# dbry/audio-resampler

Hardware: AMD Instinct MI355X
Metric: Msamples/s (out) 44.1k->48k preset -4, 8ch float32 (higher is better)
Workload: dtype i8 x 4 digits (32-bit fixed point of the f32 samples and the fp64-blended filter rows, exact i32 accumulation, one float rounding per output)

## Files before the change

### audio_resampler_amd/csrc/fir_matrix_i8.hip

```cpp
#include "fir_matrix_stream.hip.h"
#include <atomic>
#include <cstdlib>

#if !ART_WIDE

namespace {

typedef int i32x4 __attribute__ ((ext_vector_type (4)));
typedef int i32x16 __attribute__ ((ext_vector_type (16)));

constexpr int I8_KC = 32;
constexpr int I8_PITCH = 48;
constexpr int I8_COLS = 128;
constexpr int I8_MAX_PPW = 64;
constexpr int i8_ppw (int cols, int cg) { return cols / cg > I8_MAX_PPW ? I8_MAX_PPW : cols / cg; }
constexpr float I8_SCALE = 1073741824.0f;
constexpr float I8_LIMIT = 1.98f;

struct I8Geom {
    int tr;
    int cols;
    int tiles;
    int ktot;
    int g;
    int gq4;
    int super_groups;
    int sg_per_xcd;
    unsigned char *a_planes;
    unsigned long long *a_masks;
    unsigned long long *tile_masks;
    int mask_words;
    const unsigned char *x_planes;
    unsigned int *x_planes_w;
    int eb_periods, ebs;
    int eb_blocks, eb_step;
    int b0;
    int cgrp;
    int slices;
    int slice_blocks;
    unsigned int *peaks;
    unsigned int eb_plane_bytes;
    size_t x_bytes;
    int *flag; int epoch;
    int *shifts;
    unsigned char *parts;
    int rows_cached;
    int rows_table;
    double tb_base; int tb_lin, tb_w;
    unsigned int tb_n0;
    int jr_rot;
};

__device__ __forceinline__ int shift_of_peak (unsigned int bits)
{
    const int e = max ((int)(bits >> 23), 1);
    return 157 - e - ((bits & 0x7e0000u) == 0x7e0000u ? 1 : 0);
}

constexpr int I8_STAGE_THREADS = 256;
constexpr int I8_STAGE_K = 4;

__device__ __forceinline__ unsigned int digits_of (int q) { return ((unsigned int) q + 0x80808080u) ^ 0x80808080u; }

__device__ __forceinline__ long long i8_total (int s0, int s1, int s2, int s3, int s4)
{
    long long v = (long long) s0;
    v = (v << 8) + (long long) s1; v = (v << 8) + (long long) s2; v = (v << 8) + (long long) s3; v = (v << 8) + (long long) s4;
    return v;
}
__device__ __forceinline__ float i8_round (long long v, int out_exp) { return (float) __builtin_ldexp ((double) v, out_exp); }

__device__ __forceinline__ void to_planes (const unsigned int (&s) [4], unsigned int (&pl) [4])
{
    const unsigned int t01_hi = __builtin_amdgcn_perm (s [1], s [0], 0x06020703u);
    const unsigned int t01_lo = __builtin_amdgcn_perm (s [1], s [0], 0x04000501u);
    const unsigned int t23_hi = __builtin_amdgcn_perm (s [3], s [2], 0x06020703u);
    const unsigned int t23_lo = __builtin_amdgcn_perm (s [3], s [2], 0x04000501u);
    pl [0] = __builtin_amdgcn_perm (t23_hi, t01_hi, 0x05040100u);
    pl [1] = __builtin_amdgcn_perm (t23_hi, t01_hi, 0x07060302u);
    pl [2] = __builtin_amdgcn_perm (t23_lo, t01_lo, 0x05040100u);
    pl [3] = __builtin_amdgcn_perm (t23_lo, t01_lo, 0x07060302u);
}

template <bool HEAD, bool PEAK>
__device__ __forceinline__ void stage_slice (const ArtFirArgs &a, const MfmaGeom &g, const I8Geom &q, int eb, int cgi, int slice, int gb0)
{
    __shared__ unsigned int s_peak [32];
    const int tid = threadIdx.x;
    const int c = cgi * q.cgrp + (tid & (q.cgrp - 1));
    const int per_k = I8_STAGE_THREADS / q.cgrp;
    const int bl0 = slice * q.slice_blocks + tid / q.cgrp;
    const int bl_end = min ((slice + 1) * q.slice_blocks, q.eb_blocks);
    const int lin0 = 4 * (gb0 + bl0) - g.head_pad;
    const unsigned int row = (unsigned int) a.C * 4u;
    const __amdgpu_buffer_rsrc_t r_in = make_rsrc (a.in, (unsigned int)((size_t) a.in_frames * row));
    const __amdgpu_buffer_rsrc_t r_hist = make_rsrc (a.hist, (unsigned int) a.H * row);
    if (tid < 32) s_peak [tid] = 0u;
    __syncthreads ();
    if constexpr (!PEAK) {
        for (int i = tid; i < q.slices * q.cgrp; i += I8_STAGE_THREADS) {
            const int sl = i / q.cgrp, cc = i - sl * q.cgrp;
            const unsigned int pkv = q.peaks [(size_t)(eb * q.slices + sl) * a.C + cgi * q.cgrp + cc];
            if (pkv) atomicMax (&s_peak [cc], pkv);
        }
    }
    if constexpr (PEAK && !HEAD) {
        if (q.cgrp >= 4) {
            const int vpf = q.cgrp >> 2, cq = tid & (vpf - 1), per_f = I8_STAGE_THREADS / vpf;
            const int f0 = 4 * (gb0 + slice * q.slice_blocks) - g.head_pad - a.H + tid / vpf, f_end = 4 * (gb0 + bl_end) - g.head_pad - a.H;
            const unsigned int voff = (unsigned int)(f0 * a.C + cgi * q.cgrp + 4 * cq) * 4u;
            unsigned int m4 [4] = { 0u, 0u, 0u, 0u };
#pragma unroll
            for (int k = 0; k < I8_STAGE_K; ++k)
                if (f0 + k * per_f < f_end) {
                    const u32x4 x = __builtin_amdgcn_raw_buffer_load_b128 (r_in, (int) voff, (int)((unsigned int)(k * per_f) * row), 0);
                    m4 [0] = max (m4 [0], x.x & 0x7fffffffu); m4 [1] = max (m4 [1], x.y & 0x7fffffffu);
                    m4 [2] = max (m4 [2], x.z & 0x7fffffffu); m4 [3] = max (m4 [3], x.w & 0x7fffffffu);
                }
            for (int off = 32; off >= vpf; off >>= 1)
#pragma unroll
                for (int e = 0; e < 4; ++e) m4 [e] = max (m4 [e], (unsigned int) __shfl_xor ((int) m4 [e], off));
            if ((tid & 63) < vpf)
#pragma unroll
                for (int e = 0; e < 4; ++e) if (m4 [e]) atomicMax (&s_peak [4 * cq + e], m4 [e]);
            __syncthreads ();
            if (tid < q.cgrp) q.peaks [(size_t)(eb * q.slices + slice) * a.C + c] = s_peak [tid];
            return;
        }
    }
    unsigned int v [I8_STAGE_K] [4];
    unsigned int m = 0u;
    const unsigned int voff_in = (unsigned int)((lin0 - a.H) * a.C + c) * 4u;
#pragma unroll
    for (int k = 0; k < I8_STAGE_K; ++k) {
        const bool live = bl0 + k * per_k < bl_end;
#pragma unroll
        for (int t = 0; t < 4; ++t) {
            unsigned int x = 0u;
            if (live) {
                if constexpr (HEAD) {
                    const int lin = lin0 + 4 * k * per_k + t;
                    const unsigned int xi = __builtin_amdgcn_raw_buffer_load_b32 (r_in, lin >= a.H ? (int)((unsigned int)((lin - a.H) * a.C + c) * 4u) : -16, 0, 0);
                    const unsigned int xh = __builtin_amdgcn_raw_buffer_load_b32 (r_hist, lin >= 0 && lin < a.H ? (int)((unsigned int)(lin * a.C + c) * 4u) : -16, 0, 0);
                    x = xi | xh;
                }
                else x = __builtin_amdgcn_raw_buffer_load_b32 (r_in, (int) voff_in, (int)((unsigned int)(4 * k * per_k + t) * row), 0);
            }
            v [k] [t] = x;
            m = max (m, x & 0x7fffffffu);
        }
    }
    if constexpr (PEAK) {
        for (int off = 32; off >= q.cgrp; off >>= 1) m = max (m, (unsigned int) __shfl_xor ((int) m, off));
        if ((tid & 63) < q.cgrp && m) atomicMax (&s_peak [tid & (q.cgrp - 1)], m);
        __syncthreads ();
        if (tid < q.cgrp) q.peaks [(size_t)(eb * q.slices + slice) * a.C + c] = s_peak [tid];
        return;
    }
    __syncthreads ();
    const unsigned int pk = s_peak [tid & (q.cgrp - 1)];
    const int shift = shift_of_peak (pk);
    if (tid < q.cgrp && slice == 0) {
        q.shifts [eb * a.C + c] = shift;
        if (pk >= 0x7f800000u) *q.flag = q.epoch;
    }
    const __amdgpu_buffer_rsrc_t r_out = make_rsrc (q.x_planes_w + (size_t) eb * q.eb_plane_bytes, 4u * q.eb_plane_bytes);
    const unsigned int voff_out = (unsigned int)(bl0 * a.C + c) * 4u;
    const __amdgpu_buffer_rsrc_t r_head = make_rsrc (g.head, g.head ? (unsigned int) g.head_frames * row : 0u);
    const unsigned int voff_head = (unsigned int)((lin0 + g.head_pad) * a.C + c) * 4u;
#pragma unroll
    for (int k = 0; k < I8_STAGE_K; ++k) {
        if (bl0 + k * per_k < bl_end) {
            unsigned int sd [4], pl [4];
#pragma unroll
            for (int t = 0; t < 4; ++t) {
                if constexpr (HEAD) __builtin_amdgcn_raw_buffer_store_b32 (v [k] [t], r_head, (int) voff_head, (int)((unsigned int)(4 * k * per_k + t) * row), 0);
                sd [t] = digits_of (__float2int_rn (ldexpf (__uint_as_float (v [k] [t]), shift)));
            }
            to_planes (sd, pl);
#pragma unroll
            for (int pn = 0; pn < 4; ++pn) __builtin_amdgcn_raw_buffer_store_b32 (pl [pn], r_out, (int) voff_out, (int)((unsigned int) pn * q.eb_plane_bytes + (unsigned int)(k * per_k) * row), 0);
        }
    }
}

template <bool INTERP, bool PEAK>
__global__ __launch_bounds__ (I8_STAGE_THREADS)
void i8_stage_kernel (ArtFirArgs a, ArtSegTable segs, MfmaGeom g, I8Geom q)
{
    const int tid = threadIdx.x;
    const unsigned int t_wgs = 0u;
    auto slot_pos = [&] (int k) -> Pos {
        if (q.rows_table) {
            const unsigned int n = q.tb_n0 + (unsigned int) k;
            const double step = n ? (double) n / a.ratio : 0.0;
            const double off = q.tb_base + step;
            const double whole = floor (off);
            Pos t;
            double fr = off - whole;
            fr = fr * (double) a.F;
            if (INTERP) { t.fi = (int) floor (fr); t.frac = fr - (double) t.fi; }
            else { t.fi = (int) floor (fr + 0.5); t.frac = 0.0; }
            t.ip = (int) whole + q.tb_lin + q.tb_w;
            return t;
        }
        return locate<INTERP> (a, segs, a.n_begin + (unsigned int) k);
    };
    const unsigned int a_wgs = PEAK && !q.rows_cached ? t_wgs + (unsigned int)(q.tiles * q.g * q.tr) : 0u;
    auto write_tables = [&] (int st, int row) {
        const int rows_valid = min (32, g.P - st * 32);
        const Pos p0 = slot_pos (st * 32);
        const Pos p = slot_pos (st * 32 + min (row, rows_valid - 1));
        const float *h0 = a.bank + (size_t) p.fi * a.T;
        __shared__ unsigned int s_pass;
        if (row == 0) {
            if (tid == 0) s_pass = 0u;
            __syncthreads ();
            if (tid == 0) {
                g.tile_w0 [3 * st] = p0.ip - a.T / 2 + 1;
                if (st == 0) a.fix_count [0] = 0;
            }
            if (!INTERP && !a.lowpass && tid < rows_valid) {
                const Pos pq = slot_pos (st * 32 + tid);
                if ((pq.fi % a.F) == 0) atomicOr (&s_pass, 1u << tid);
            }
            __syncthreads ();
            if (tid == 0) { g.tile_w0 [3 * st + 1] = (int) s_pass; g.tile_w0 [3 * st + 2] = 0; }
        }
        if (tid == 0) { g.canon_ip [st * 32 + row] = p.ip; g.canon_fi [st * 32 + row] = p.fi; g.canon_frac [st * 32 + row] = p.frac; }
        float *dst = g.eff + (size_t)(st * 32 + row) * g.ktot;
        for (int k = tid; k < g.ktot; k += 256) {
            const int tap = k - (p.ip - p0.ip);
            float cf = 0.0f;
            if (tap >= 0 && tap < a.T) {
                if (INTERP) {
                    const double left = (double) h0 [tap] * (1.0 - p.frac);
                    const double right = (double) h0 [tap + a.T] * p.frac;
                    cf = (float)(left + right);
                }
                else cf = h0 [tap];
            }
            dst [k] = cf;
        }
    };
    if (blockIdx.x < t_wgs) {
        write_tables ((int) blockIdx.x >> 5, (int) blockIdx.x & 31);
        return;
    }
    if (blockIdx.x < a_wgs) {
        const int ab = (int)(blockIdx.x - t_wgs);
        const int variant = ab / q.tr, row = ab - variant * q.tr;
        const int st = variant / q.g, jr = variant - st * q.g;
        if (jr == 0 && (q.tr == 32 ? st : 2 * st + (row >> 5)) < g.slot_tiles) write_tables (q.tr == 32 ? st : 2 * st + (row >> 5), row & 31);
        const int rows_valid = min (q.tr, g.P - st * q.tr);
        const Pos p0 = slot_pos (st * q.tr);
        const Pos p = slot_pos (st * q.tr + min (row, rows_valid - 1));
        const float *h0 = a.bank + (size_t) p.fi * a.T;
        const int r = max (p0.ip - a.T / 2 + 1 + jr * g.Q + g.head_pad, 0) & 3;
        const int shift = p.ip - p0.ip + r;
        bool bad = false;
        __shared__ unsigned long long s_mask, s_mask1;
        if (tid == 0) { s_mask = 0ull; s_mask1 = 0ull; }
        __syncthreads ();
        unsigned long long mine = 0ull, mine1 = 0ull;
        const int chunk_bytes = q.tr * 128, plane_bytes = q.tr * 32, half_bytes = q.tr * 16;
        unsigned char *base = q.a_planes + (size_t) variant * (q.ktot / I8_KC) * chunk_bytes + row * 16;
        for (int k4 = tid * 4; k4 < q.ktot; k4 += 1024) {
            unsigned int s [4], pl [4];
#pragma unroll
            for (int t = 0; t < 4; ++t) {
                const int tap = k4 + t - shift;
                double v = 0.0;
                if (row < rows_valid && tap >= 0 && tap < a.T) {
                    if (INTERP) {
                        const double left = (double) h0 [tap] * (1.0 - p.frac);
                        const double right = (double) h0 [tap + a.T] * p.frac;
                        v = left + right;
                    }
                    else v = (double) h0 [tap];
                }
                if (!(fabs (v) < (double) I8_LIMIT)) { bad = true; v = 0.0; }
                s [t] = digits_of ((int) rint (v * (double) I8_SCALE));
            }
            to_planes (s, pl);
#pragma unroll
            for (int pn = 0; pn < 4; ++pn) *reinterpret_cast<unsigned int *> (base + (size_t)(k4 >> 5) * chunk_bytes + pn * plane_bytes + ((k4 >> 4) & 1) * half_bytes + (k4 & 15)) = pl [pn];
            if (pl [0]) mine |= 1ull << (k4 >> 5);
            if (pl [1]) mine1 |= 1ull << (k4 >> 5);
        }
        if (mine) atomicOr (&s_mask, mine);
        if (mine1) atomicOr (&s_mask1, mine1);
        __syncthreads ();
        if (tid == 0) { q.a_masks [variant * q.tr + row] = s_mask; q.a_masks [q.mask_words + variant * q.tr + row] = s_mask1; }
        if (bad) *q.flag = q.epoch;
        return;
    }
    const int groups = a.C / q.cgrp;
    const int xid = (int)(blockIdx.x - a_wgs);
    if (!PEAK && xid >= q.ebs * groups * q.slices) {
        const int e = (xid - q.ebs * groups * q.slices) * I8_STAGE_THREADS + tid, halves = q.tr / 32;
        if (e < q.tiles * q.g * halves) {
            unsigned long long m = 0ull, m1 = 0ull;
            for (int r = 0; r < 32; ++r) { m |= q.a_masks [(e / halves) * q.tr + (e % halves) * 32 + r]; m1 |= q.a_masks [q.mask_words + (e / halves) * q.tr + (e % halves) * 32 + r]; }
            q.tile_masks [e] = m; q.tile_masks [q.tiles * q.g * halves + e] = m1;
        }
        return;
    }
    const int slice = xid % q.slices, xb = xid / q.slices, eb = xb / groups, cgi = xb - eb * groups;
    const int gb0 = q.b0 + eb * q.eb_step;
    if (4 * (gb0 + slice * q.slice_blocks) - g.head_pad < max (a.H, g.head_frames - g.head_pad)) stage_slice<true, PEAK> (a, g, q, eb, cgi, slice, gb0);
    else stage_slice<false, PEAK> (a, g, q, eb, cgi, slice, gb0);
}

template <int VEC> struct PlaneLoad;
template <> struct PlaneLoad<1> { static __device__ __forceinline__ void load (unsigned int *dst, __amdgpu_buffer_rsrc_t r, unsigned int off, unsigned int soff) {
    dst [0] = __builtin_amdgcn_raw_buffer_load_b32 (r, (int) off, (int) soff, 0); } };
template <> struct PlaneLoad<2> { static __device__ __forceinline__ void load (unsigned int *dst, __amdgpu_buffer_rsrc_t r, unsigned int off, unsigned int soff) {
    u32x2 v = __builtin_amdgcn_raw_buffer_load_b64 (r, (int) off, (int) soff, 0); dst [0] = v.x; dst [1] = v.y; } };
template <> struct PlaneLoad<4> { static __device__ __forceinline__ void load (unsigned int *dst, __amdgpu_buffer_rsrc_t r, unsigned int off, unsigned int soff) {
    u32x4 v = __builtin_amdgcn_raw_buffer_load_b128 (r, (int) off, (int) soff, 0); dst [0] = v.x; dst [1] = v.y; dst [2] = v.z; dst [3] = v.w; } };

template <int CG, bool PASS>
__device__ __forceinline__ void stand_by_tiles (const ArtFirArgs &a, const MfmaGeom &g, int wgs_per_xcd, float (&As_) [2] [32 * MF_LD], float (&Bs_) [2] [MF_COLS * MF_LD])
{
    constexpr int THREADS = 2 * MF_THREADS;
    constexpr int PPW = MF_COLS / CG > MF_MAX_PPW ? MF_MAX_PPW : MF_COLS / CG;
    constexpr int NCOLS = PPW * CG;
    const int tid = threadIdx.x, lane = tid & 63, wave = tid >> 6;
    const bool loader = wave >= 4;
    const int pt = tid & (MF_THREADS - 1);
    (void) THREADS;
#include "fir_matrix_stream_body.inc"
}

__device__ __forceinline__ int i8_table_entry (const int *table, int i) { return __builtin_amdgcn_readfirstlane (table [i]); }
__device__ __forceinline__ int i8_table_entry (const __attribute__ ((address_space (4))) int *table, int i) { return table [i]; }

template <int CG, bool PASS>
__global__ __launch_bounds__ (2 * MF_THREADS) __attribute__ ((amdgpu_waves_per_eu (4, 4)))
void fir_i8_stream_kernel (ArtFirArgs a, MfmaGeom g, I8Geom q, int wgs_per_xcd)
{
    constexpr int THREADS = 2 * MF_THREADS;
    constexpr int PPW = i8_ppw (I8_COLS, CG);
    constexpr int NCOLS = PPW * CG;
    __shared__ __attribute__ ((aligned (16))) unsigned char As_ [2] [4] [32 * I8_PITCH];
    __shared__ __attribute__ ((aligned (16))) unsigned char Bs_ [2] [4] [I8_COLS * I8_PITCH];

    const int tid = threadIdx.x, lane = tid & 63, wave = tid >> 6;
    const bool loader = wave >= 4;
    const int pt = tid & (MF_THREADS - 1);

#define I8_PART 1
#include "fir_i8_tile32.inc"

    if (NCOLS < I8_COLS)
        for (int e = tid; e < 2 * 4 * (I8_COLS - NCOLS) * I8_PITCH / 4; e += THREADS) {
            const int per = (I8_COLS - NCOLS) * I8_PITCH / 4, bp = e / per, r = e - bp * per;
            reinterpret_cast<unsigned int *> (&Bs_ [bp >> 2] [bp & 3] [NCOLS * I8_PITCH]) [r] = 0u;
        }

    if (loader) {
        constexpr int VEC = CG >= 4 ? 4 : (CG == 2 ? 2 : 1);
        constexpr int VPF = CG / VEC, VPP = (I8_KC / 4) * VPF, NB = (PPW * VPP) / MF_THREADS;
        static_assert ((PPW * VPP) % MF_THREADS == 0 && NB >= 1, "every staging thread moves NB vectors per plane and chunk");
        constexpr unsigned int A_STEP = 4096u, B_STEP = (I8_KC / 4) * CG * 4u;
        const int a_plane = pt >> 6, a_half = (pt >> 5) & 1, a_row = pt & 31;
        const unsigned int a_off0 = (unsigned int) pt * 16u;
        const int adst = a_plane * (32 * I8_PITCH) + a_row * I8_PITCH + a_half * 16;
        unsigned int boff [NB], bdel [NB]; int bdst [NB], bper [NB];
#pragma unroll
        for (int u = 0; u < NB; ++u) {
            const int v = pt + u * MF_THREADS;
            const int m = v / VPP, rem = v % VPP, kb = rem / VPF, cv = rem % VPF;
            boff [u] = (unsigned int)((m * q.gq4 + kb) * CG + cv * VEC) * 4u;
            bdst [u] = (m * CG + cv * VEC) * I8_PITCH + kb * 4;
            bper [u] = m * q.g;
            bdel [u] = 0u;
        }
        unsigned int ra0 [2] [4], rb0 [2] [4] [NB * VEC];
        const int *tile_w0 = g.tile_w0;

#define I8_PART 2
#include "fir_i8_tile32.inc"
        auto fetch_next = [&] (auto set_tag) {
            constexpr int SET = decltype (set_tag)::value;
            if (f_live) {
                const unsigned int sa = (unsigned int) f_chunk * A_STEP, sb = min ((unsigned int) f_chunk * B_STEP, fb_bytes);
                const __amdgpu_buffer_rsrc_t ra_ = make_rsrc (fa_base + sa, fa_bytes - sa), rb_ = make_rsrc (fb_base + sb, fb_bytes - sb);
                {
                    u32x4 v = __builtin_amdgcn_raw_buffer_load_b128 (ra_, (int) a_off0, 0, 0);
                    ra0 [SET] [0] = v.x; ra0 [SET] [1] = v.y; ra0 [SET] [2] = v.z; ra0 [SET] [3] = v.w;
                }
#pragma unroll
                for (int pn = 0; pn < 4; ++pn)
#pragma unroll
                    for (int u = 0; u < NB; ++u) PlaneLoad<VEC>::load (&rb0 [SET] [pn] [u * VEC], rb_, boff [u] + bdel [u], (unsigned int) pn * q.eb_plane_bytes);
                if (++f_chunk == nchunks) { f_chunk = 0; open_tile (); }
            }
        };
        auto commit = [&] (auto set_tag) {
            constexpr int SET = decltype (set_tag)::value;
            i32x4 v;
#pragma unroll
            for (int i = 0; i < 4; ++i) v [i] = (int) ra0 [SET] [i];
            *reinterpret_cast<i32x4 *> (&As_ [SET] [0] [adst]) = v;
#pragma unroll
            for (int pn = 0; pn < 4; ++pn)
#pragma unroll
                for (int u = 0; u < NB; ++u)
#pragma unroll
                    for (int e = 0; e < VEC; ++e) *reinterpret_cast<unsigned int *> (&Bs_ [SET] [pn] [bdst [u] + e * I8_PITCH]) = rb0 [SET] [pn] [u * VEC + e];
        };
        const std::integral_constant<int, 0> S0 {};
        const std::integral_constant<int, 1> S1 {};

        const int total = my_tiles * nchunks;
        open_tile ();
        fetch_next (S0); fetch_next (S1);
        commit (S0); fetch_next (S0);
        __syncthreads ();
        for (int c = 0; c < total; c += 2) {
            commit (S1); fetch_next (S1);
            __syncthreads ();
            if (c + 1 < total) {
                commit (S0); fetch_next (S0);
                __syncthreads ();
            }
        }
        return;
    }

    {
        const unsigned int hw_id = __builtin_amdgcn_s_getreg ((4 - 1) << 11 | 16 << 6 | 4);
        if (hw_id & 1u) __builtin_amdgcn_s_setprio (3); else __builtin_amdgcn_s_setprio (0);
    }
    const int aoff = (lane & 31) * I8_PITCH + (lane >> 5) * 16;
    const int col = wave * 32 + (lane & 31);
    const bool col_live = col < NCOLS;
    const int jl = col / CG, c = col - jl * CG;
    const int boff = col * I8_PITCH + (lane >> 5) * 16;
    const unsigned int out_off = (unsigned int)((jl * q.g * g.P + 4 * (lane >> 5)) * CG + c) * 4u;

    __syncthreads ();
    int qn = 0;
    for (int within = rank; within < tiles_per_xcd; within += wgs_per_xcd) {
        int st, j0;
        if (!tile_at (within, st, j0)) continue;
#define I8_PART 3
#include "fir_i8_tile32.inc"

        for (int ch = 0; ch < nchunks; ++ch, ++qn) {
            const unsigned char *Ab = &As_ [0] [0] [0] + (qn & 1) * (int) sizeof (As_ [0]) + aoff;
            const unsigned char *Bb = &Bs_ [0] [0] [0] + (qn & 1) * (int) sizeof (Bs_ [0]) + boff;
            i32x4 av [4], bv [4];
#pragma unroll
            for (int pn = 0; pn < 4; ++pn) {
                av [pn] = *reinterpret_cast<const i32x4 *> (Ab + pn * (32 * I8_PITCH));
                bv [pn] = *reinterpret_cast<const i32x4 *> (Bb + pn * (I8_COLS * I8_PITCH));
            }
            __builtin_amdgcn_sched_group_barrier (0x100, 8, 0);
            __syncthreads ();
#define I8_PART 4
#include "fir_i8_tile32.inc"
        }
// ... 364 lines not shown
#pragma unroll
            for (int r = 0; r < 16; ++r) tot [h] [r] = i8_total (acc [h] [0] [r], acc [h] [1] [r], acc [h] [2] [r], acc [h] [3] [r], acc [h] [4] [r]);
        if (c0 != 0 || c1 != nch) {
            constexpr int COHERENT = 1 | 16;
            const int t = within - D * W;
            auto owner_of = [&] (int chunk) {
                int r = (int)(((long long) chunk * Weff) / Ct);
                while (r + 1 < Weff && ((r + 1) * Ct) / Weff <= chunk) ++r;
                return r;
            };
            const int r_first = owner_of (t * nch), r_last = owner_of ((t + 1) * nch - 1);
            const unsigned int wave_bytes = 16u * 64u * 16u;
            unsigned int *count = sl.arrivals + ((size_t)(xcd * SL_MAX_SK + t) * 8 + wave);
            unsigned int before = 0u;
            bool look = k == nseg - 1 && k != D;
            if (look) {
                if (lane == 0) before = __hip_atomic_load (count, __ATOMIC_RELAXED, __HIP_MEMORY_SCOPE_AGENT);
                before = (unsigned int) __builtin_amdgcn_readfirstlane ((int) before);
                look = before == (unsigned int)(r_last - r_first);
            }
            if (!look) {
                const int which = k == D ? 0 : 1;
                const __amdgpu_buffer_rsrc_t rs_part = make_rsrc (sl.parts + ((size_t)((xcd * W + rank) * 2 + which) * 8 + wave) * wave_bytes, wave_bytes);
#pragma unroll
                for (int r = 0; r < 16; ++r) {
                    u32x4 v;
                    const unsigned long long x0 = (unsigned long long) tot [0] [r], x1 = (unsigned long long) tot [1] [r];
                    v.x = (unsigned int) x0; v.y = (unsigned int)(x0 >> 32); v.z = (unsigned int) x1; v.w = (unsigned int)(x1 >> 32);
                    __builtin_amdgcn_raw_buffer_store_b128 (v, rs_part, (r * 64 + lane) * 16, 0, COHERENT);
                }
                asm volatile ("s_waitcnt vmcnt(0)" ::: "memory");
                if (lane == 0) before = __hip_atomic_fetch_add (count, 1u, __ATOMIC_RELAXED, __HIP_MEMORY_SCOPE_AGENT);
                before = (unsigned int) __builtin_amdgcn_readfirstlane ((int) before);
            }
            if (before != (unsigned int)(r_last - r_first)) continue;
            if (lane == 0) __hip_atomic_store (count, 0u, __ATOMIC_RELAXED, __HIP_MEMORY_SCOPE_AGENT);
            for (int rr = r_first; rr <= r_last; ++rr) {
                if (rr == rank) continue;
                const int which = (rr * Ct) / Weff / nch == t ? 0 : 1;
                const __amdgpu_buffer_rsrc_t rs_part = make_rsrc (sl.parts + ((size_t)((xcd * W + rr) * 2 + which) * 8 + wave) * wave_bytes, wave_bytes);
                u32x4 v [16];
#pragma unroll
                for (int r = 0; r < 16; ++r) v [r] = __builtin_amdgcn_raw_buffer_load_b128 (rs_part, (r * 64 + lane) * 16, 0, COHERENT);
#pragma unroll
                for (int r = 0; r < 16; ++r) {
                    tot [0] [r] += (long long)((unsigned long long) v [r].x | (unsigned long long) v [r].y << 32);
                    tot [1] [r] += (long long)((unsigned long long) v [r].z | (unsigned long long) v [r].w << 32);
                }
            }
        }
        const int out_exp = -14 - shift_v;
        const unsigned int n_tile = a.n_begin + (unsigned int) j0 * g.P + (unsigned int)(st * 64);
        const int rows_valid = min (64, g.P - st * 64);
        const size_t left = (size_t)(a.n_end - n_tile) * CG * 4;
        const __amdgpu_buffer_rsrc_t rs_out = make_rsrc (a.out + (size_t) n_tile * CG, left > 0xffffff00ull ? 0xffffff00u : (unsigned int) left);
        float y [2] [16];
#pragma unroll
        for (int h = 0; h < 2; ++h) {
            const unsigned int pass_rows = PASS && 2 * st + h < g.slot_tiles ? (unsigned int) tile_w0 [3 * (2 * st + h) + 1] : 0u;
#pragma unroll
            for (int r = 0; r < 16; ++r) {
                y [h] [r] = i8_round (tot [h] [r], out_exp);
                if constexpr (PASS) {
                    const int i = h * 32 + (r & 3) + 8 * (r >> 2) + 4 * (lane >> 5);
                    if ((pass_rows >> (i & 31)) & 1u)
                        y [h] [r] = load_frame (a, INT_MIN, g.canon_ip [st * 64 + i] + g.w_shift + g.canon_fi [st * 64 + i] / a.F + (j0 + jl * q.g) * g.Q, c);
                }
            }
        }
        {
            int lane_e = lane;
            asm volatile ("" : "+v" (lane_e));
            const int qm = lane_e & 3;
            const int lo = a.n_skip != 0 && j0 == 0 && wave == 0 ? a.n_skip - st * 64 : 0;
            const int col_e = wave * 32 + (lane_e & 31), jl_e = col_e / CG, c_e = col_e - jl_e * CG;
            const unsigned int q_off = (unsigned int)((((jl_e << g_log2) * g.P) + 4 * (lane_e >> 5) + qm) * CG + (c_e & ~3)) * 4u;
#pragma unroll
            for (int h = 0; h < 2; ++h)
#pragma unroll
                for (int rb = 0; rb < 4; ++rb) {
                    unsigned int t [4];
#pragma unroll
                    for (int u = 0; u < 4; ++u) t [u] = __float_as_uint (y [h] [4 * rb + u]);
#pragma unroll
                    for (int pr = 0; pr < 4; pr += 2) {
                        const unsigned int send = (qm & 1) ? t [pr] : t [pr + 1];
                        const unsigned int recv = (unsigned int) __builtin_amdgcn_mov_dpp ((int) send, 0xB1, 0xf, 0xf, true);
                        if (qm & 1) t [pr] = recv; else t [pr + 1] = recv;
                    }
#pragma unroll
                    for (int pr = 0; pr < 2; ++pr) {
                        const unsigned int send = (qm & 2) ? t [pr] : t [pr + 2];
                        const unsigned int recv = (unsigned int) __builtin_amdgcn_mov_dpp ((int) send, 0x4E, 0xf, 0xf, true);
                        if (qm & 2) t [pr] = recv; else t [pr + 2] = recv;
                    }
                    u32x4 v; v.x = t [0]; v.y = t [1]; v.z = t [2]; v.w = t [3];
                    const int i_const = h * 32 + 8 * rb;
                    const int i = i_const + 4 * (lane >> 5) + qm;
                    const unsigned int off = i < rows_valid && (i >= lo || (lane & 31) >= CG) ? q_off + (unsigned int)(i_const * CG) * 4u : 0xfffffff0u;
                    __builtin_amdgcn_raw_buffer_store_b128 (v, rs_out, (int) off, 0, 0);
                }
        }
    }
    asm volatile ("s_waitcnt vmcnt(0)" ::: "memory");
}


}

bool artfir_i8_slab_enabled ()
{
    static const bool on = [] { const char *e = getenv ("ARTAMD_I8_SLAB"); return !(e && *e == '0'); } ();
    return on;
}
static int i8_slab_min_tiles ()
{
    static const int v = [] { const char *e = getenv ("ARTAMD_I8_SLAB_MIN"); return e && *e ? atoi (e) : 24; } ();
    return v;
}

static size_t i8_layout (const ArtFirArgs *a, const MfmaGeom &g, int cgt, I8Geom &q, char *base, unsigned int outputs = 0)
{
    if (!cgt || g.tile_rows != 32 || (g.ktot % I8_KC)) return 0;
    const unsigned int total = outputs ? outputs + (unsigned int) g.P : a->n_end - a->n_begin, periods = (total + g.P - 1) / g.P;
    q.g = (g.Q % 4 == 0) ? 1 : (g.Q % 2 == 0) ? 2 : 4;
    q.tr = 32; q.cols = I8_COLS; q.rows_cached = 0; q.jr_rot = 0; q.rows_table = 0; q.tb_base = 0.0; q.tb_lin = q.tb_w = 0; q.tb_n0 = 0u;
    if (artfir_i8_slab_enabled () && cgt >= 4) {
        const int ppw64 = i8_ppw (SL_COLS, cgt);
        const int sgs = (int)((periods + (unsigned int)(q.g * ppw64) - 1) / (unsigned int)(q.g * ppw64));
        const int per_xcd = ((sgs + 7) / 8) * q.g * ((g.P + 63) / 64);
        if (per_xcd >= i8_slab_min_tiles ()) { q.tr = 64; q.cols = SL_COLS; }
    }
    for (;;) {
        const int shift_max = (int)((q.tr - 1.0) * g.Q / g.P) + 2;
        q.ktot = ((a->T + shift_max + 3 + I8_KC - 1) / I8_KC) * I8_KC;
        if (q.tr == 64 && (q.ktot / I8_KC < 4 || q.ktot / I8_KC > 64)) { q.tr = 32; q.cols = I8_COLS; continue; }
        break;
    }
    q.tiles = (g.P + q.tr - 1) / q.tr;
    const int ppw = i8_ppw (q.cols, cgt);
    q.gq4 = q.g * g.Q / 4;
    q.super_groups = (int)((periods + (unsigned int)(q.g * ppw) - 1) / (unsigned int)(q.g * ppw));
    q.sg_per_xcd = (q.super_groups + 7) / 8;
    if (q.ktot / I8_KC > 64) return 0;
    {
        const int unit = 16 * q.g * g.Q;
        const int k = (9408 + unit / 2) / unit;
        q.eb_periods = 16 * q.g * (k > 1 ? k : 1);
    }
    q.eb_step = q.eb_periods * g.Q / 4;
    const int over_blocks = (g.Q + 2 + q.ktot + 3 + 3) / 4 + 2;
    q.eb_blocks = q.eb_step + over_blocks;
    q.ebs = (int)((periods + (unsigned int) q.eb_periods - 1) / (unsigned int) q.eb_periods);
    q.cgrp = a->C < 8 ? a->C : 8;
    q.slice_blocks = I8_STAGE_K * I8_STAGE_THREADS / q.cgrp;
    q.slices = (q.eb_blocks + q.slice_blocks - 1) / q.slice_blocks;
    q.eb_plane_bytes = (unsigned int) q.eb_blocks * (unsigned int) a->C * 4u;
    q.x_bytes = (size_t) q.ebs * 4 * q.eb_plane_bytes;
    q.b0 = 0;
    const size_t a_bytes = (size_t) q.tiles * q.g * (q.ktot / I8_KC) * (size_t)(q.tr * 128);
    const size_t masks = 2 * ((size_t) q.tiles * q.g * q.tr * 8 + (size_t) q.tiles * q.g * (q.tr / 32) * 8), shifts = (size_t) q.ebs * a->C * 4;
    const size_t teams = (size_t) q.ebs * q.slices * a->C * 4;
    const size_t head = (ART_I8_HEAD_BYTES + masks + teams + shifts + 255) & ~(size_t) 255;
    q.flag = (int *) base; q.epoch = 0;
    q.a_masks = (unsigned long long *)(base + ART_I8_HEAD_BYTES);
    q.mask_words = q.tiles * q.g * q.tr;
    q.tile_masks = q.a_masks + 2 * (size_t) q.mask_words;
    q.peaks = (unsigned int *)(base + ART_I8_HEAD_BYTES + masks);
    q.shifts = (int *)(base + ART_I8_HEAD_BYTES + masks + teams);
    q.a_planes = (unsigned char *) base + head;
    q.x_planes_w = (unsigned int *)(base + head + a_bytes); q.x_planes = (const unsigned char *) q.x_planes_w;
    q.parts = q.tr == 64 ? (unsigned char *) base + ((head + a_bytes + q.x_bytes + 255) & ~(size_t) 255) : nullptr;
    return q.tr == 64 ? ((head + a_bytes + q.x_bytes + 255) & ~(size_t) 255) + (size_t) 8 * SL_WGS * 2 * SL_PART_BYTES : head + a_bytes + q.x_bytes;
}

size_t artfir_i8_bytes (const ArtFirArgs *a, const MfmaGeom &g, int cgt, unsigned int outputs)
{
    I8Geom q;
    return i8_layout (a, g, cgt, q, nullptr, outputs ? outputs : 1u);
}

namespace {

struct RowsSetPtrs {
    unsigned long long *a_masks, *tile_masks; unsigned char *a_planes;
    float *eff; double *canon_frac; int *canon_ip, *canon_fi, *tile_w0;
};
static size_t rows_set_layout (const MfmaGeom &g, const I8Geom &q, char *base, RowsSetPtrs *out)
{
    size_t off = 0;
    auto take = [&] (size_t bytes) { const size_t at = off; off = (off + bytes + 255) & ~(size_t) 255; return at; };
    const size_t rows32 = (size_t) g.slot_tiles * 32;
    const size_t o_masks = take (2 * (size_t) q.tiles * q.g * q.tr * 8), o_tm = take (2 * (size_t) q.tiles * q.g * (q.tr / 32) * 8);
    const size_t o_planes = take ((size_t) q.tiles * q.g * (q.ktot / I8_KC) * (size_t)(q.tr * 128));
    const size_t o_eff = take (rows32 * g.ktot * sizeof (float)), o_frac = take (rows32 * sizeof (double));
    const size_t o_ip = take (rows32 * sizeof (int)), o_fi = take (rows32 * sizeof (int)), o_w0 = take ((size_t) 3 * g.slot_tiles * sizeof (int));
    if (out && base) {
        out->a_masks = (unsigned long long *)(base + o_masks); out->tile_masks = (unsigned long long *)(base + o_tm); out->a_planes = (unsigned char *)(base + o_planes);
        out->eff = (float *)(base + o_eff); out->canon_frac = (double *)(base + o_frac); out->canon_ip = (int *)(base + o_ip); out->canon_fi = (int *)(base + o_fi);
        out->tile_w0 = (int *)(base + o_w0);
    }
    return off;
}

}

extern "C" {
size_t arthip_fir_rows_cache_bytes (void) { return sizeof (ArtRowsCache); }
void arthip_fir_rows_cache_reset (void *cache)
{
    ArtRowsCache *rc = (ArtRowsCache *) cache;
    if (rc) { for (int k = 0; k < 4; ++k) rc->valid [k] = 0; rc->f_valid = 0; }
}
void arthip_fir_rows_cache_free (void *cache)
{
    ArtRowsCache *rc = (ArtRowsCache *) cache;
    if (rc) {
        free (rc->c_ph); free (rc->c_ip); free (rc->c_fi); rc->c_ph = nullptr; rc->c_ip = rc->c_fi = nullptr; rc->cap = 0; rc->canon_valid = 0;
    }
}
}

size_t artfir_i8_rows_bytes (const ArtFirArgs *a, const MfmaGeom &g, int cgt, unsigned int outputs)
{
    I8Geom q;
    if (!i8_layout (a, g, cgt, q, nullptr, outputs ? outputs : 1u)) return 0;
    return (size_t)(4 / q.g) * (rows_set_layout (g, q, nullptr, nullptr) + 4096);
}

namespace {

typedef void (*I8TileKernel) (ArtFirArgs, MfmaGeom, I8Geom, int);
typedef void (*I8SlabKernel) (ArtFirArgs, MfmaGeom, I8Geom, I8Slab);
#define I8_PICK(KERNEL, CGT) (pass ? KERNEL<CGT, true> : KERNEL<CGT, false>)
I8TileKernel i8_tile_kernel (int cgt, bool pass)
{
    switch (cgt) {
        case 32: return I8_PICK (fir_i8_dma_kernel, 32);
        case 16: return I8_PICK (fir_i8_dma_kernel, 16);
        case 8: return I8_PICK (fir_i8_dma_kernel, 8);
        case 4: return I8_PICK (fir_i8_dma_kernel, 4);
        case 2: return I8_PICK (fir_i8_stream_kernel, 2);
        default: return I8_PICK (fir_i8_stream_kernel, 1);
    }
}
I8SlabKernel i8_slab_kernel (int cgt, bool pass)
{
    switch (cgt) {
        case 32: return I8_PICK (fir_i8_slab_kernel, 32);
        case 16: return I8_PICK (fir_i8_slab_kernel, 16);
        case 8: return I8_PICK (fir_i8_slab_kernel, 8);
        default: return I8_PICK (fir_i8_slab_kernel, 4);
    }
}
#undef I8_PICK

}

int artfir_i8_launch (const ArtFirArgs *a_in, const ArtSegTable *segs, const MfmaGeom &g_in, int cgt, unsigned int roll_blocks, hipStream_t st)
{
    static std::atomic<int> launches {0};
    I8Geom q;
    if (!a_in->planes) return 0;
    ArtFirArgs a_v = *a_in; const ArtFirArgs *a = &a_v;
    MfmaGeom g = g_in;

    ArtRowsCache *rc = artfir_rows_cache_enabled () && a_in->rows ? (ArtRowsCache *) a_in->rows_cache : nullptr;
    HostPos pos0;
    int slot0 = 0, w = 0;
    if (!artfir_rows_canonical (a_in, segs, g.P, g.Q, rc, &pos0, &slot0, &w)) rc = nullptr;
    if (rc && rc->c_ip [0] + w - a_in->T / 2 + 1 + g.head_pad < 0) rc = nullptr;
    if (rc) {
        a_v.n_begin = a_in->n_begin + (unsigned int)(g.P - slot0); a_v.n_end = a_in->n_end + (unsigned int) g.P;
        a_v.out = a_in->out - (size_t) g.P * a_in->C; a_v.n_skip = slot0;
    }
    size_t need = i8_layout (a, g, cgt, q, (char *) a_in->planes);
    auto without_rows = [&] () { rc = nullptr; a_v = *a_in; need = i8_layout (a, g, cgt, q, (char *) a_in->planes); };
    if (rc && (!need || need > a_in->planes_bytes)) without_rows ();
    if (!need || need > a_in->planes_bytes) return 0;

    bool build_from_table = false;
    int set = -1;
    if (rc) {
        const size_t set_bytes = rows_set_layout (g, q, nullptr, nullptr);
        const int nsets = 4 / q.g;
        const bool same = rc->lowpass == a_in->lowpass && rc->tr == q.tr && rc->ktot == q.ktot && rc->tiles == q.tiles && rc->g == q.g && rc->slot_tiles == g.slot_tiles &&
                          rc->ktot32 == g.ktot && rc->set_bytes == set_bytes && rc->nsets == nsets;
        if (artfir_f32_set_bytes (g) + (size_t) nsets * (set_bytes + 4096) > a_in->rows_bytes) {
            without_rows ();
            if (!need || need > a_in->planes_bytes) return 0;
        }
        else {
            if (!same) {
                for (int k = 0; k < 4; ++k) rc->valid [k] = 0;
                rc->lowpass = a_in->lowpass; rc->tr = q.tr; rc->ktot = q.ktot; rc->tiles = q.tiles; rc->g = q.g; rc->slot_tiles = g.slot_tiles; rc->ktot32 = g.ktot;
                rc->set_bytes = set_bytes; rc->nsets = nsets; rc->victim = 0;
            }
            const int step = 4 / q.g;
            for (int k = 0; k < nsets && set < 0; ++k) {
                if (!rc->valid [k] || ((w - rc->w_build [k]) % step) != 0) continue;
                const int dw = w - rc->w_build [k];
                for (int r = 0; r < q.g; ++r) if ((((long long) r * g.Q - dw) & 3) == 0) { set = k; g.w_shift = dw; q.jr_rot = r; q.rows_cached = 1; break; }
            }
            if (set < 0) {
                for (int k = 0; k < nsets && set < 0; ++k) if (!rc->valid [k]) set = k;
                if (set < 0) { set = rc->victim; rc->victim = (rc->victim + 1) % nsets; }
                rc->valid [set] = 1; rc->w_build [set] = w;
                g.w_shift = 0; q.jr_rot = 0; q.rows_cached = 0; build_from_table = true;
            }
            RowsSetPtrs sp;
            rows_set_layout (g, q, (char *) a_in->rows + artfir_f32_set_bytes (g) + (size_t) set * (set_bytes + 4096), &sp);
            q.a_masks = sp.a_masks; q.tile_masks = sp.tile_masks; q.a_planes = sp.a_planes;
            g.eff = sp.eff; g.canon_frac = sp.canon_frac; g.canon_ip = sp.canon_ip; g.canon_fi = sp.canon_fi; g.tile_w0 = sp.tile_w0;
        }
    }
    q.rows_table = build_from_table ? 1 : 0;
    if (build_from_table) { q.tb_base = rc->c_base; q.tb_lin = rc->c_lin; q.tb_n0 = rc->c_n0; q.tb_w = w; }
    {   static const bool trace = [] { const char *e = getenv ("ARTAMD_ROWS_TRACE"); return e && *e == '1'; } ();
        if (trace) fprintf (stderr, "rows: launch n %u..%u  cache %s  slot0 %d  w %d  set %d  %s  w_shift %d rot %d  tr %d  ph0 %.12f ip0 %d\n", a_in->n_begin, a_in->n_end,
                            rc ? "on" : "off", slot0, w, set, rc ? (build_from_table ? "BUILD" : "hit") : "-", g.w_shift, q.jr_rot, q.tr, pos0.ph, pos0.ip);
    }
    if (a_in->rows_masks_out) *a_in->rows_masks_out = (void *) q.a_masks;

    int ep = ++launches;
    if (ep <= 0) { launches = 1; ep = 1; }
    q.epoch = ep;
    if (a->fixed_out) { a->fixed_out [0] = ep; a->fixed_out [1] = q.tiles * q.g * q.tr; a->fixed_out [2] = q.ktot / I8_KC; a->fixed_out [3] = q.tr == 64 ? 3 : cgt >= 4 ? 2 : 1; }

    {
        const int ip = rc ? rc->c_ip [0] + w : pos0.ip;
        const int la = ip - a->T / 2 + 1 + g.head_pad;
        q.b0 = (la > 0 ? la : 0) >> 2;
    }
    const unsigned int x_wgs = (unsigned int)(q.ebs * (a->C / q.cgrp) * q.slices);
    const dim3 pgrid (x_wgs + (q.rows_cached ? 0u : (unsigned int)(q.tiles * q.g * q.tr))),
               xgrid (x_wgs + (q.rows_cached ? 0u : (unsigned int)((q.tiles * q.g * (q.tr / 32) + I8_STAGE_THREADS - 1) / I8_STAGE_THREADS)));
    if (a->interpolate) {
        hipLaunchKernelGGL ((i8_stage_kernel<true, true>), pgrid, dim3 (I8_STAGE_THREADS), 0, st, *a, *segs, g, q);
        hipLaunchKernelGGL ((i8_stage_kernel<true, false>), xgrid, dim3 (I8_STAGE_THREADS), 0, st, *a, *segs, g, q);
    }
    else {
        hipLaunchKernelGGL ((i8_stage_kernel<false, true>), pgrid, dim3 (I8_STAGE_THREADS), 0, st, *a, *segs, g, q);
        hipLaunchKernelGGL ((i8_stage_kernel<false, false>), xgrid, dim3 (I8_STAGE_THREADS), 0, st, *a, *segs, g, q);
    }
    if (a->ev_start) arthip_event_record (a->ev_start, (void *) st);

    const int tiles_per_xcd = q.sg_per_xcd * q.g * q.tiles;
    const int resident = 62;
    const int wgs_per_xcd = tiles_per_xcd < resident ? tiles_per_xcd : resident;
    const bool fixup = artfir_pass_fixup_wanted (a);
    const bool pass = !a->interpolate && !a->lowpass && !fixup;
    if (q.tr == 64) {
        I8Slab sl;
        sl.wgs_per_xcd = SL_WGS;
        sl.parts = q.parts;
        sl.arrivals = (unsigned int *)((char *) a->planes + ART_I8_FLAG_BYTES);
        {
            const int ppw = i8_ppw (q.cols, cgt);
            const unsigned int n_out = a->n_end - a->n_begin;
            for (int x = 0; x < 8; ++x) {
                int live = 0; bool prefix = true;
                for (int w = 0; w < tiles_per_xcd; ++w) {
                    const int stt = w % q.tiles, t2 = w / q.tiles, jr = t2 % q.g, sg = x * q.sg_per_xcd + t2 / q.g;
                    const bool ok = sg < q.super_groups && (unsigned long long)(sg * q.g * ppw + jr) * (unsigned int) g.P + (unsigned int)(stt * 64) < n_out;
                    if (ok) { if (live != w) prefix = false; ++live; }
                }
                if (!prefix) return 0;
                sl.live [x] = live;
            }
        }
        const dim3 wgrid ((unsigned int)(8 * SL_WGS));
        hipLaunchKernelGGL (i8_slab_kernel (cgt, pass), wgrid, dim3 (SL_THREADS), 0, st, *a, g, q, sl);
        if (a->ev_stop) arthip_event_record (a->ev_stop, (void *) st);
        if (fixup && artfir_pass_fixup (a, g, st)) return -1;
        return 1;
    }
    const dim3 sgrid ((unsigned int)(8 * wgs_per_xcd) + roll_blocks);
    hipLaunchKernelGGL (i8_tile_kernel (cgt, pass), sgrid, dim3 (2 * MF_THREADS), 0, st, *a, g, q, wgs_per_xcd);
    if (a->ev_stop) arthip_event_record (a->ev_stop, (void *) st);
    if (fixup && artfir_pass_fixup (a, g, st)) return -1;
    return 1;
}

#endif
```

Baseline: 80930.

## Widen channel groups to 32 with vectorised quantise and shuffle peak gather

Raises the channel group size to 32 and scales stage threads per workgroup up to 1024 for wide channel counts. Adds a path that quantises four channels per thread using 128-bit loads and stores when the group has at least 16 channels. It also replaces the per-element atomic peak gather with a wavefront shuffle reduction followed by fewer shared atomics. For 8-channel input the group size and thread count are unchanged, so mainly the reduction rewrite applies.

```diff
diff --git a/audio_resampler_amd/csrc/fir_matrix_i8.hip b/audio_resampler_amd/csrc/fir_matrix_i8.hip
--- a/audio_resampler_amd/csrc/fir_matrix_i8.hip
+++ b/audio_resampler_amd/csrc/fir_matrix_i8.hip
@@ -57,8 +57,9 @@
     return 157 - e - ((bits & 0x7e0000u) == 0x7e0000u ? 1 : 0);
 }
 
-constexpr int I8_STAGE_THREADS = 256;
 constexpr int I8_STAGE_K = 4;
+constexpr int i8_stage_threads (int cgrp) { return cgrp > 16 ? 1024 : cgrp > 8 ? 512 : 256; }
+constexpr int I8_VECTOR_QUANTISE_MIN = 16;
 
 __device__ __forceinline__ unsigned int digits_of (int q) { return ((unsigned int) q + 0x80808080u) ^ 0x80808080u; }
 
@@ -82,13 +83,13 @@
     pl [3] = __builtin_amdgcn_perm (t23_lo, t01_lo, 0x07060302u);
 }
 
-template <bool HEAD, bool PEAK>
+template <bool HEAD, bool PEAK, int THREADS>
 __device__ __forceinline__ void stage_slice (const ArtFirArgs &a, const MfmaGeom &g, const I8Geom &q, int eb, int cgi, int slice, int gb0)
 {
     __shared__ unsigned int s_peak [32];
     const int tid = threadIdx.x;
     const int c = cgi * q.cgrp + (tid & (q.cgrp - 1));
-    const int per_k = I8_STAGE_THREADS / q.cgrp;
+    const int per_k = THREADS / q.cgrp;
     const int bl0 = slice * q.slice_blocks + tid / q.cgrp;
     const int bl_end = min ((slice + 1) * q.slice_blocks, q.eb_blocks);
     const int lin0 = 4 * (gb0 + bl0) - g.head_pad;
@@ -98,15 +99,16 @@
     if (tid < 32) s_peak [tid] = 0u;
     __syncthreads ();
     if constexpr (!PEAK) {
-        for (int i = tid; i < q.slices * q.cgrp; i += I8_STAGE_THREADS) {
-            const int sl = i / q.cgrp, cc = i - sl * q.cgrp;
-            const unsigned int pkv = q.peaks [(size_t)(eb * q.slices + sl) * a.C + cgi * q.cgrp + cc];
-            if (pkv) atomicMax (&s_peak [cc], pkv);
+        for (int i0 = 0; i0 < q.slices * q.cgrp; i0 += THREADS) {
+            const int i = i0 + tid, sl = i / q.cgrp;
+            unsigned int pkv = sl < q.slices ? q.peaks [(size_t)(eb * q.slices + sl) * a.C + c] : 0u;
+            for (int off = 32; off >= q.cgrp; off >>= 1) pkv = max (pkv, (unsigned int) __shfl_xor ((int) pkv, off));
+            if ((tid & 63) < q.cgrp && pkv) atomicMax (&s_peak [tid & (q.cgrp - 1)], pkv);
         }
     }
     if constexpr (PEAK && !HEAD) {
         if (q.cgrp >= 4) {
-            const int vpf = q.cgrp >> 2, cq = tid & (vpf - 1), per_f = I8_STAGE_THREADS / vpf;
+            const int vpf = q.cgrp >> 2, cq = tid & (vpf - 1), per_f = THREADS / vpf;
             const int f0 = 4 * (gb0 + slice * q.slice_blocks) - g.head_pad - a.H + tid / vpf, f_end = 4 * (gb0 + bl_end) - g.head_pad - a.H;
             const unsigned int voff = (unsigned int)(f0 * a.C + cgi * q.cgrp + 4 * cq) * 4u;
             unsigned int m4 [4] = { 0u, 0u, 0u, 0u };
@@ -125,6 +127,51 @@
                 for (int e = 0; e < 4; ++e) if (m4 [e]) atomicMax (&s_peak [4 * cq + e], m4 [e]);
             __syncthreads ();
             if (tid < q.cgrp) q.peaks [(size_t)(eb * q.slices + slice) * a.C + c] = s_peak [tid];
+            return;
+        }
+    }
+    if constexpr (!PEAK && !HEAD) {
+        if (q.cgrp >= I8_VECTOR_QUANTISE_MIN) {
+            static_assert (I8_STAGE_K % 4 == 0, "a vector unit is four scalar ones");
+            const int vpf = q.cgrp >> 2, cq = tid & (vpf - 1), per_b = THREADS / vpf;
+            const int blv = slice * q.slice_blocks + tid / vpf;
+            const unsigned int voff = (unsigned int)((4 * (gb0 + blv) - g.head_pad - a.H) * a.C + cgi * q.cgrp + 4 * cq) * 4u;
+            u32x4 x [I8_STAGE_K / 4] [4];
+#pragma unroll
+            for (int k = 0; k < I8_STAGE_K / 4; ++k)
+#pragma unroll
+                for (int t = 0; t < 4; ++t) {
+                    x [k] [t] = u32x4 { 0u, 0u, 0u, 0u };
+                    if (blv + k * per_b < bl_end) x [k] [t] = __builtin_amdgcn_raw_buffer_load_b128 (r_in, (int) voff, (int)((unsigned int)(4 * k * per_b + t) * row), 0);
+                }
+            __syncthreads ();
+            int sh [4];
+#pragma unroll
+            for (int e = 0; e < 4; ++e) sh [e] = shift_of_peak (s_peak [4 * cq + e]);
+            if (tid < q.cgrp && slice == 0) {
+                const unsigned int pk = s_peak [tid];
+                q.shifts [eb * a.C + c] = shift_of_peak (pk);
+                if (pk >= 0x7f800000u) *q.flag = q.epoch;
+            }
+            const __amdgpu_buffer_rsrc_t r_out = make_rsrc (q.x_planes_w + (size_t) eb * q.eb_plane_bytes, 4u * q.eb_plane_bytes);
+            const unsigned int voff_out = (unsigned int)(blv * a.C + cgi * q.cgrp + 4 * cq) * 4u;
+#pragma unroll
+            for (int k = 0; k < I8_STAGE_K / 4; ++k) {
+                if (blv + k * per_b < bl_end) {
+                    unsigned int pl [4] [4];
+#pragma unroll
+                    for (int e = 0; e < 4; ++e) {
+                        unsigned int sd [4];
+#pragma unroll
+                        for (int t = 0; t < 4; ++t) sd [t] = digits_of (__float2int_rn (ldexpf (__uint_as_float (x [k] [t] [e]), sh [e])));
+                        to_planes (sd, pl [e]);
+                    }
+#pragma unroll
+                    for (int pn = 0; pn < 4; ++pn)
+                        __builtin_amdgcn_raw_buffer_store_b128 (u32x4 { pl [0] [pn], pl [1] [pn], pl [2] [pn], pl [3] [pn] }, r_out, (int) voff_out,
+                                                                (int)((unsigned int) pn * q.eb_plane_bytes + (unsigned int)(k * per_b) * row), 0);
+                }
+            }
             return;
         }
     }
@@ -184,8 +231,8 @@
     }
 }
 
-template <bool INTERP, bool PEAK>
-__global__ __launch_bounds__ (I8_STAGE_THREADS)
+template <bool INTERP, bool PEAK, int THREADS>
+__global__ __launch_bounds__ (THREADS)
 void i8_stage_kernel (ArtFirArgs a, ArtSegTable segs, MfmaGeom g, I8Geom q)
 {
     const int tid = threadIdx.x;
@@ -229,7 +276,7 @@
         }
         if (tid == 0) { g.canon_ip [st * 32 + row] = p.ip; g.canon_fi [st * 32 + row] = p.fi; g.canon_frac [st * 32 + row] = p.frac; }
         float *dst = g.eff + (size_t)(st * 32 + row) * g.ktot;
-        for (int k = tid; k < g.ktot; k += 256) {
+        for (int k = tid; k < g.ktot; k += THREADS) {
             const int tap = k - (p.ip - p0.ip);
             float cf = 0.0f;
             if (tap >= 0 && tap < a.T) {
@@ -265,7 +312,7 @@
         unsigned long long mine = 0ull, mine1 = 0ull;
         const int chunk_bytes = q.tr * 128, plane_bytes = q.tr * 32, half_bytes = q.tr * 16;
         unsigned char *base = q.a_planes + (size_t) variant * (q.ktot / I8_KC) * chunk_bytes + row * 16;
-        for (int k4 = tid * 4; k4 < q.ktot; k4 += 1024) {
+        for (int k4 = tid * 4; k4 < q.ktot; k4 += 4 * THREADS) {
             unsigned int s [4], pl [4];
 #pragma unroll
             for (int t = 0; t < 4; ++t) {
@@ -298,7 +345,7 @@
     const int groups = a.C / q.cgrp;
     const int xid = (int)(blockIdx.x - a_wgs);
     if (!PEAK && xid >= q.ebs * groups * q.slices) {
-        const int e = (xid - q.ebs * groups * q.slices) * I8_STAGE_THREADS + tid, halves = q.tr / 32;
+        const int e = (xid - q.ebs * groups * q.slices) * THREADS + tid, halves = q.tr / 32;
         if (e < q.tiles * q.g * halves) {
             unsigned long long m = 0ull, m1 = 0ull;
             for (int r = 0; r < 32; ++r) { m |= q.a_masks [(e / halves) * q.tr + (e % halves) * 32 + r]; m1 |= q.a_masks [q.mask_words + (e / halves) * q.tr + (e % halves) * 32 + r]; }
@@ -308,8 +355,16 @@
     }
     const int slice = xid % q.slices, xb = xid / q.slices, eb = xb / groups, cgi = xb - eb * groups;
     const int gb0 = q.b0 + eb * q.eb_step;
-    if (4 * (gb0 + slice * q.slice_blocks) - g.head_pad < max (a.H, g.head_frames - g.head_pad)) stage_slice<true, PEAK> (a, g, q, eb, cgi, slice, gb0);
-    else stage_slice<false, PEAK> (a, g, q, eb, cgi, slice, gb0);
+    if (4 * (gb0 + slice * q.slice_blocks) - g.head_pad < max (a.H, g.head_frames - g.head_pad)) stage_slice<true, PEAK, THREADS> (a, g, q, eb, cgi, slice, gb0);
+    else stage_slice<false, PEAK, THREADS> (a, g, q, eb, cgi, slice, gb0);
+}
+
+template <bool INTERP, bool PEAK>
+void i8_stage_launch (unsigned int threads, dim3 grid, hipStream_t st, const ArtFirArgs &a, const ArtSegTable &segs, const MfmaGeom &g, const I8Geom &q)
+{
+    if (threads == 1024) hipLaunchKernelGGL ((i8_stage_kernel<INTERP, PEAK, 1024>), grid, dim3 (1024), 0, st, a, segs, g, q);
+    else if (threads == 512) hipLaunchKernelGGL ((i8_stage_kernel<INTERP, PEAK, 512>), grid, dim3 (512), 0, st, a, segs, g, q);
+    else hipLaunchKernelGGL ((i8_stage_kernel<INTERP, PEAK, 256>), grid, dim3 (256), 0, st, a, segs, g, q);
 }
 
 template <int VEC> struct PlaneLoad;
@@ -980,8 +1035,8 @@
     const int over_blocks = (g.Q + 2 + q.ktot + 3 + 3) / 4 + 2;
     q.eb_blocks = q.eb_step + over_blocks;
     q.ebs = (int)((periods + (unsigned int) q.eb_periods - 1) / (unsigned int) q.eb_periods);
-    q.cgrp = a->C < 8 ? a->C : 8;
-    q.slice_blocks = I8_STAGE_K * I8_STAGE_THREADS / q.cgrp;
+    q.cgrp = a->C < 32 ? a->C : 32;
+    q.slice_blocks = I8_STAGE_K * i8_stage_threads (q.cgrp) / q.cgrp;
     q.slices = (q.eb_blocks + q.slice_blocks - 1) / q.slice_blocks;
     q.eb_plane_bytes = (unsigned int) q.eb_blocks * (unsigned int) a->C * 4u;
     q.x_bytes = (size_t) q.ebs * 4 * q.eb_plane_bytes;
@@ -1161,16 +1216,11 @@
         q.b0 = (la > 0 ? la : 0) >> 2;
     }
     const unsigned int x_wgs = (unsigned int)(q.ebs * (a->C / q.cgrp) * q.slices);
+    const unsigned int sthreads = (unsigned int) i8_stage_threads (q.cgrp);
     const dim3 pgrid (x_wgs + (q.rows_cached ? 0u : (unsigned int)(q.tiles * q.g * q.tr))),
-               xgrid (x_wgs + (q.rows_cached ? 0u : (unsigned int)((q.tiles * q.g * (q.tr / 32) + I8_STAGE_THREADS - 1) / I8_STAGE_THREADS)));
-    if (a->interpolate) {
-        hipLaunchKernelGGL ((i8_stage_kernel<true, true>), pgrid, dim3 (I8_STAGE_THREADS), 0, st, *a, *segs, g, q);
-        hipLaunchKernelGGL ((i8_stage_kernel<true, false>), xgrid, dim3 (I8_STAGE_THREADS), 0, st, *a, *segs, g, q);
-    }
-    else {
-        hipLaunchKernelGGL ((i8_stage_kernel<false, true>), pgrid, dim3 (I8_STAGE_THREADS), 0, st, *a, *segs, g, q);
-        hipLaunchKernelGGL ((i8_stage_kernel<false, false>), xgrid, dim3 (I8_STAGE_THREADS), 0, st, *a, *segs, g, q);
-    }
+               xgrid (x_wgs + (q.rows_cached ? 0u : ((unsigned int)(q.tiles * q.g * (q.tr / 32)) + sthreads - 1) / sthreads));
+    if (a->interpolate) { i8_stage_launch<true, true> (sthreads, pgrid, st, *a, *segs, g, q); i8_stage_launch<true, false> (sthreads, xgrid, st, *a, *segs, g, q); }
+    else { i8_stage_launch<false, true> (sthreads, pgrid, st, *a, *segs, g, q); i8_stage_launch<false, false> (sthreads, xgrid, st, *a, *segs, g, q); }
     if (a->ev_start) arthip_event_record (a->ev_start, (void *) st);
 
     const int tiles_per_xcd = q.sg_per_xcd * q.g * q.tiles;
```

After: 79870. 1.3% lower.
